# edouardlp/Mask-RCNN-CoreML

Hardware: AMD Instinct MI355X
Metric: images/sec (1024x1024, COCO-80) (higher is better)
Workload: dtype f32x3

## Files before the change

### mask-rcnn-coreml_amd/csrc/kernels_conv_halo.hip

```cpp
#include "conv_device.h"

#include <stdlib.h>
#include <map>
#include <mutex>
#include <string>
#include <utility>

namespace mrcnn {

ConvScratch* conv_current_scratch();

static int env_int_halo(const char* name, int dflt) { const char* e = knob_env(name); return e ? atoi(e) : dflt; }

static constexpr int HALO_MAX_SLOT = 640;
static constexpr unsigned HALO_OOB = 0xC0000000u;
enum { HALO_GEO_LINEAR = 0,
       HALO_GEO_ROW = 1,
       HALO_GEO_2ROWS = 2,
       HALO_GEO_4ROWS = 3 };

typedef unsigned u32x4 __attribute__((ext_vector_type(4)));
typedef unsigned u32x2 __attribute__((ext_vector_type(2)));

struct HaloArgs {
    ConvArgs a;
    const void* wgt_halo;
    int NH;
    int geo;
    int ecols;
    int pitch;
    int img_skew;
    int tiles_row, tiles_img;
    int n_tiles;
    const void* head_w;
    const float* head_bias;
    float* head_out; float* head_out2;
    long head_out_sB, head_out_sP, head_out2_sB, head_out2_sP;
    int head_split, head_cols;
    float head_mul;
    ConvArgs t;
    const void* t_w;
    void* t_park;
};

template <int PARTS>
__device__ __forceinline__ void split4(const u32x4 v, u32x2 (&out)[PARTS])
{
    const float a[4] = {__uint_as_float(v[0]), __uint_as_float(v[1]), __uint_as_float(v[2]), __uint_as_float(v[3])};
#pragma unroll
    for (int p = 0; p < 2; ++p) {
        const uint32_t h2 = cvt_pk_rne(a[2 * p], a[2 * p + 1]);
        float r0, r1;
        asm("v_fma_mix_f32 %0, %1, -1.0, %2 op_sel:[0,0,0] op_sel_hi:[1,0,0]" : "=v"(r0) : "v"(h2), "v"(a[2 * p]));
        asm("v_fma_mix_f32 %0, %1, -1.0, %2 op_sel:[1,0,0] op_sel_hi:[1,0,0]" : "=v"(r1) : "v"(h2), "v"(a[2 * p + 1]));
        const uint32_t m2 = cvt_pk_rne(r0, r1);
        out[0][p] = h2;
        out[1][p] = m2;
        if constexpr (PARTS == 3) {
            float q0, q1;
            asm("v_fma_mix_f32 %0, %1, -1.0, %2 op_sel:[0,0,0] op_sel_hi:[1,0,0]" : "=v"(q0) : "v"(m2), "v"(r0));
            asm("v_fma_mix_f32 %0, %1, -1.0, %2 op_sel:[1,0,0] op_sel_hi:[1,0,0]" : "=v"(q1) : "v"(m2), "v"(r1));
            out[2][p] = cvt_pk_rne(q0, q1);
        }
    }
}

template <int PARTS, int TN, bool HEAD = false, bool DBG = false, int TM = 2, int MAXPC = 5, bool TAIL = false, int WN = 4>
__global__ __launch_bounds__(512, 2) void k_conv_halo(const HaloArgs ha)
{
    const ConvArgs& a = ha.a;
    static_assert(WN == 4 || (WN == 2 && TM == 1 && TN == 1 && !HEAD && !TAIL) || (WN == 1 && TM == 1 && TN == 2 && !HEAD && !TAIL),
                  "wave arrangement 2 x 4; 4 x 2 with one accumulator per wave; 8 x 1 with two (256 x 64 tiles)");
    static_assert(!HEAD || TN == 2, "the fused head walks the K groups of 256-column tiles");
    static_assert(!TAIL || (TM == 2 && TN == 2 && !HEAD), "the fused tail needs the whole 128 x 256 tile in one block");
    static_assert(MAXPC >= 2 && MAXPC <= 5, "staging pieces per thread");
    constexpr int WMR = 8 / WN;
    constexpr int BM = WMR * TM * 32, BN = WN * TN * 32;
    constexpr int PLANE = (HALO_MAX_SLOT + 1) * 32;
    constexpr int PBUF = PARTS * PLANE;
    constexpr int STAGE = 8 * 32 * 36 * 4;
    constexpr int HPART = 4 * BM * 32 * 4;
    constexpr int HRUN = HEAD ? BM * 32 * 4 : 0;
    constexpr int PLANES_ = 2 * PBUF > PBUF + STAGE ? 2 * PBUF : PBUF + STAGE;
    constexpr int TAILPL = 16 * 64 * 32;
    constexpr int TAILN = 1024;
    constexpr int TPLANES = TAIL ? PARTS * TAILPL + STAGE : 0;
    constexpr int PLANES__ = HEAD && HPART > PLANES_ ? HPART : PLANES_;
    constexpr int PLANES = TPLANES > PLANES__ ? TPLANES : PLANES__;
    constexpr int TAB1 = TAIL ? 2 * TAILN * 4 : 0;
    __shared__ __attribute__((aligned(16))) unsigned char smem[PLANES + 2 * 2 * BN * 4 + HRUN + TAB1];
    unsigned char* const planes = smem;
    float* const s_tab0 = reinterpret_cast<float*>(smem + PLANES);
    float* const h_run = reinterpret_cast<float*>(smem + PLANES + 2 * 2 * BN * 4);
    float* const tab1 = reinterpret_cast<float*>(smem + PLANES + 2 * 2 * BN * 4 + HRUN);

    const int t = threadIdx.x;
    const int lane = t & 63;
    const int wave = __builtin_amdgcn_readfirstlane(t >> 6);
    const int wm = WN == 4 ? wave >> 2 : (WN == 2 ? wave >> 1 : wave), wn = WN == 4 ? wave & 3 : (WN == 2 ? wave & 1 : 0);
    const int l31 = lane & 31, kk = lane >> 5;
    const int ohw = a.OH * a.OW;
    const int NH = ha.NH, NS = NH * 9;

    const int T = HEAD ? a.tiles_m : ha.n_tiles;
    const int n_inner = HEAD ? a.tiles_n : 1;
    const int nb = gridDim.x;
    const int bid = blockIdx.x;
    int t_first, t_end, t_step;
    {
        const int q = T >> 3, r8 = T & 7;
        const int xcd = bid & 7, j = bid >> 3;
        const int lo = xcd < r8 ? xcd * (q + 1) : r8 * (q + 1) + (xcd - r8) * q;
        const int cnt = q + (xcd < r8 ? 1 : 0);
        const int per = nb >> 3;
        t_first = lo + j; t_end = lo + cnt; t_step = per;
        if (nb < 8) { t_first = bid; t_end = T; t_step = nb; }
    }

    typedef unsigned srd_t __attribute__((ext_vector_type(4)));
    srd_t srdB;
    {
        const unsigned long long wa = (unsigned long long)(uintptr_t)ha.wgt_halo;
        srdB[0] = __builtin_amdgcn_readfirstlane((unsigned)wa);
        srdB[1] = __builtin_amdgcn_readfirstlane((unsigned)(wa >> 32) & 0xffffu);
        srdB[2] = 0xffffffffu;
        srdB[3] = 0x00020000u;
    }
    const unsigned vlane16 = (unsigned)lane * 16u;
    srd_t srdT;
    {
        const unsigned long long ta_ = (unsigned long long)(uintptr_t)(TAIL ? ha.t_w : ha.wgt_halo);
        srdT[0] = __builtin_amdgcn_readfirstlane((unsigned)ta_);
        srdT[1] = __builtin_amdgcn_readfirstlane((unsigned)(ta_ >> 32) & 0xffffu);
        srdT[2] = 0xffffffffu;
        srdT[3] = 0x00020000u;
    }
    if constexpr (TAIL) {
        const float4 one = make_float4(1.f, 1.f, 1.f, 1.f), zero = make_float4(0.f, 0.f, 0.f, 0.f);
        if (t < TAILN / 4) {
            *reinterpret_cast<float4*>(&tab1[4 * t]) = ha.t.scale ? *reinterpret_cast<const float4*>(ha.t.scale + 4 * t) : one;
            *reinterpret_cast<float4*>(&tab1[TAILN + 4 * t]) = ha.t.shift ? *reinterpret_cast<const float4*>(ha.t.shift + 4 * t) : zero;
        }
    }
    const int dbg = DBG ? a.dbg : 0;
    const bool dbg_nodma = dbg & 1, dbg_nobar = dbg & 2, dbg_nords = dbg & 4, dbg_nomma = dbg & 8, dbg_nostage = dbg & 16;
    const bool dbg_noloads = dbg & 64, dbg_nosplit = dbg & 128, dbg_nowrite = dbg & 256;

    int tile_par = 0;
    for (int unit = t_first; unit < t_end; unit += t_step)
    for (int inner = 0; inner < n_inner; ++inner, tile_par ^= 1) {
        const int mt = HEAD ? unit : unit / a.tiles_n, nt = HEAD ? inner : unit - mt * a.tiles_n;
        const int n0 = nt * BN;
        float* const s_tab = s_tab0 + tile_par * 2 * BN;
        const int Hp = a.H + 2;
        const int pitch = ha.pitch, ecols = ha.ecols;
        int m0, b0, gy_first, col0, rows;
        if (ha.geo == HALO_GEO_2ROWS || ha.geo == HALO_GEO_4ROWS) {
            const int trows = ha.geo == HALO_GEO_2ROWS ? 2 : 4;
            b0 = mt / ha.tiles_img;
            const int r = mt - b0 * ha.tiles_img, rp = r / ha.tiles_row, cb = r - rp * ha.tiles_row;
            m0 = b0 * ohw + trows * rp * a.OW + 64 * cb;
            gy_first = b0 * Hp + trows * rp + 1;
            col0 = 64 * cb - 1;
            rows = trows + 2;
        } else {
            m0 = mt * BM;
            const int m_last = (m0 + BM - 1 < a.M ? m0 + BM - 1 : a.M - 1);
            b0 = m0 / ohw;
            const int rem0 = m0 - b0 * ohw, oh0 = rem0 / a.OW, ow0 = rem0 - oh0 * a.OW;
            const int b1 = m_last / ohw, rem1 = m_last - b1 * ohw, oh1 = rem1 / a.OW;
            gy_first = b0 * Hp + oh0 + 1;
            const int gy_last = b1 * Hp + oh1 + 1;
            col0 = ha.geo == HALO_GEO_ROW ? ow0 - 1 : -1;
            rows = gy_last - gy_first + 3;
        }
        const int npx = rows * ecols;
        srd_t srdA;
        {
            const unsigned long long ia = (unsigned long long)(uintptr_t)(static_cast<const float*>(a.in) + (long)b0 * a.in_sB);
            const unsigned long long rest = (unsigned long long)(a.B - b0) * (unsigned long long)a.in_sB * 4ull;
            srdA[0] = __builtin_amdgcn_readfirstlane((unsigned)ia);
            srdA[1] = __builtin_amdgcn_readfirstlane((unsigned)(ia >> 32) & 0xffffu);
            srdA[2] = __builtin_amdgcn_readfirstlane((unsigned)(rest < 0x80000000ull ? rest : 0x80000000ull));
            srdA[3] = 0x00020000u;
        }
        unsigned p_off[MAXPC], p_lds[MAXPC];
#pragma unroll
        for (int i = 0; i < MAXPC; ++i) {
            const int j = t + 512 * i;
            const int px = j >> 2, qt = j & 3;
            const int r = px / ecols, c = px - r * ecols;
            const int gy = gy_first - 1 + r;
            const int b = gy / Hp, y = gy - b * Hp - 1;
            const int x = col0 + c;
            const bool ok = px < npx && (unsigned)y < (unsigned)a.H && (unsigned)x < (unsigned)a.W && b < a.B;
            p_off[i] = ok ? (unsigned)(((long)(b - b0) * a.in_sB + (long)y * a.in_sH + (long)x * a.in_sW + qt * 4) * 4) : HALO_OOB;
            if (DBG && (a.dbg & 32)) p_off[i] = (unsigned)((px & 63) * 1024 + qt * 16);
            const int slot = r * pitch + c + (b - b0) * ha.img_skew;
            p_lds[i] = px < npx ? (unsigned)(slot * 32 + (((qt >> 1) ^ ((slot >> 3) & 1)) << 4) + (qt & 1) * 8) : (unsigned)(HALO_MAX_SLOT * 32 + qt * 8);
        }
        int base_idx[TM];
        int wave_row0;
        if (ha.geo == HALO_GEO_2ROWS || ha.geo == HALO_GEO_4ROWS) {
            if constexpr (WN == 4) {
                wave_row0 = m0 + wm * a.OW;
#pragma unroll
                for (int i = 0; i < TM; ++i) base_idx[i] = wm * pitch + i * 32 + l31;
            } else {
                wave_row0 = m0 + (wm >> 1) * a.OW + (wm & 1) * 32;
                base_idx[0] = (wm >> 1) * pitch + (wm & 1) * 32 + l31;
            }
        } else {
            wave_row0 = m0 + wm * (TM * 32);
            const int ow0 = col0 + 1;
#pragma unroll
            for (int i = 0; i < TM; ++i) {
                const int m = wave_row0 + i * 32 + l31;
                const int mm = m < a.M ? m : a.M - 1;
                const int b = mm / ohw, rem = mm - b * ohw, oh = rem / a.OW, ow = rem - oh * a.OW;
                base_idx[i] = ha.geo == HALO_GEO_ROW ? (ow - ow0) : (b * Hp + oh + 1 - gy_first) * pitch + ow + (b - b0) * ha.img_skew;
            }
        }
        unsigned sob[TN];
#pragma unroll
        for (int j = 0; j < TN; ++j) sob[j] = (unsigned)(((size_t)(n0 / 32 + wn * TN + j) * NS) * 1024u);

        if (t < BN / 2) {
            const int c = (t < BN / 4 ? t : t - BN / 4) * 4;
            const float* src = t < BN / 4 ? a.scale : a.shift;
            const float fill = t < BN / 4 ? 1.0f : 0.0f;
            *reinterpret_cast<float4*>(&s_tab[(t < BN / 4 ? 0 : BN) + c]) =
                src ? *reinterpret_cast<const float4*>(src + n0 + c) : make_float4(fill, fill, fill, fill);
        }

#define HALO_LOAD(I) if constexpr ((I) < MAXPC) asm volatile("buffer_load_dwordx4 %0, %1, %2, 0 offen" : "=v"(st[(I) < MAXPC ? (I) : 0]) : "v"(p_off[(I) < MAXPC ? (I) : 0]), "s"(srdA) : "memory");
#define HALO_LOADS()  { HALO_LOAD(0) HALO_LOAD(1) HALO_LOAD(2) HALO_LOAD(3) HALO_LOAD(4) }
#define HALO_ADVANCE() { _Pragma("unroll") for (int i = 0; i < MAXPC; ++i) p_off[i] += (p_off[i] < HALO_OOB ? 64u : 0u); }
#define HALO_PIN1(I)  if constexpr ((I) < MAXPC) asm volatile("" : "+v"(st[(I) < MAXPC ? (I) : 0]));
#define HALO_PIN()    { HALO_PIN1(0) HALO_PIN1(1) HALO_PIN1(2) HALO_PIN1(3) HALO_PIN1(4) }
#define HALO_WRITE1(BUF, I_)                                                                                     \
    if constexpr ((I_) < MAXPC) {                                                                                \
        constexpr int I = (I_) < MAXPC ? (I_) : 0;                                                               \
        u32x2 parts[PARTS];                                                                                      \
        if (DBG && dbg_nosplit) { _Pragma("unroll") for (int p = 0; p < PARTS; ++p) { parts[p][0] = st[I][0]; parts[p][1] = st[I][p]; } } \
        else split4<PARTS>(st[I], parts);                                                                        \
        if (DBG && dbg_nowrite) { _Pragma("unroll") for (int p = 0; p < PARTS; ++p) asm volatile("" ::"v"(parts[p])); } \
        else {                                                                                                   \
            _Pragma("unroll") for (int p = 0; p < PARTS; ++p)                                                    \
                *reinterpret_cast<u32x2*>(planes + (BUF) * PBUF + p * PLANE + p_lds[I]) = parts[p];              \
        }                                                                                                        \
    }
#define HALO_WRITE(BUF) { HALO_WRITE1(BUF, 0) HALO_WRITE1(BUF, 1) HALO_WRITE1(BUF, 2) HALO_WRITE1(BUF, 3) HALO_WRITE1(BUF, 4) }
#define HALO_BLOAD(BV, STEP_)                                                                                    \
    {                                                                                                            \
        _Pragma("unroll") for (int j = 0; j < TN; ++j) {                                                         \
            const unsigned so_ = sob[j] + (unsigned)(STEP_) * 1024u;                                             \
            asm volatile("buffer_load_dwordx4 %0, %1, %2, %3 offen" : "=v"(BV[j]) : "v"(vlane16), "s"(srdB), "s"(so_) : "memory"); \
        }                                                                                                        \
    }
#define HALO_BPIN(BV) { _Pragma("unroll") for (int j = 0; j < TN; ++j) asm volatile("" : "+v"(BV[j])); }
        u32x4 st[MAXPC];
        u32x4 bv0[TN], bv1[TN], bv2[TN], bv3[TN];

        HALO_LOADS()
        HALO_ADVANCE()
        HALO_BLOAD(bv0, 0)
        HALO_BLOAD(bv1, 1)
        HALO_BLOAD(bv2, 2)
        asm volatile("s_waitcnt vmcnt(0)" ::: "memory");
        HALO_PIN()
        HALO_BPIN(bv0)
        HALO_BPIN(bv1)
        HALO_BPIN(bv2)
        HALO_WRITE(0)
        __syncthreads();

        f32x16 acc[TM][TN];
#pragma unroll
        for (int i = 0; i < TM; ++i)
#pragma unroll
            for (int j = 0; j < TN; ++j)
#pragma unroll
                for (int e = 0; e < 16; ++e) acc[i][j][e] = 0.0f;

#define HALO_AFRAGS(AV, PB_, TAP_)                                                                               \
    {                                                                                                            \
        _Pragma("unroll") for (int i = 0; i < TM; ++i) {                                                         \
            const int idx_ = base_idx[i] + ((TAP_) / 3) * pitch + ((TAP_) % 3);                                  \
            const unsigned a_addr_ = (unsigned)(idx_ << 5) + (unsigned)(((kk << 4) ^ ((idx_ << 1) & 16)));       \
            _Pragma("unroll") for (int p = 0; p < PARTS; ++p) AV[i][p] = *reinterpret_cast<const uint4*>(planes + (PB_) * PBUF + p * PLANE + a_addr_); \
        }                                                                                                        \
    }
#define HALO_STEP(BVC, BVN3, TAP, PB)                                                                            \
    {                                                                                                            \
          \
        if (!(DBG && dbg_nodma)) HALO_BLOAD(BVN3, step + 3 < NS ? step + 3 : NS - 1)                             \
        if ((TAP) == 0 && next_slab && !(DBG && dbg_noloads)) { HALO_LOADS() HALO_ADVANCE() }                    \
        if (!(DBG && dbg_nomma)) {                                                                               \
        _Pragma("unroll") for (int p = 0; p < PARTS; ++p)                                                        \
            _Pragma("unroll") for (int i = 0; i < TM; ++i)                                                       \
                _Pragma("unroll") for (int j = 0; j < TN; ++j)                                                   \
                    acc[i][j] = __builtin_amdgcn_mfma_f32_32x32x16_f16(__builtin_bit_cast(f16x8, BVC[j]), __builtin_bit_cast(f16x8, av[i][p]), acc[i][j], 0, 0, 0); \
        }                                                                                                        \
                                 \
        if (!(DBG && dbg_nords)) {                                                                               \
            if ((TAP) == 8) HALO_AFRAGS(av, (PB) ^ 1, 0)                                                         \
            else HALO_AFRAGS(av, PB, ((TAP) + 1) % 9)                                                            \
        }                                                                                                        \
            \
        if ((TAP) == 4 && next_slab) { HALO_PIN() HALO_WRITE1((PB) ^ 1, 0) HALO_WRITE1((PB) ^ 1, 4) }            \
        if ((TAP) == 5 && next_slab) HALO_WRITE1((PB) ^ 1, 1)                                                    \
        if ((TAP) == 6 && next_slab) HALO_WRITE1((PB) ^ 1, 2)                                                    \
        if ((TAP) == 7 && next_slab) HALO_WRITE1((PB) ^ 1, 3)                                                    \
        if (DBG && (dbg_nodma || dbg_noloads)) asm volatile("s_waitcnt vmcnt(0)" ::: "memory");                  \
        else if ((TAP) <= 2 && next_slab) asm volatile("s_waitcnt vmcnt(%0)" ::"n"(2 * TN + MAXPC) : "memory");  \
        else asm volatile("s_waitcnt vmcnt(%0)" ::"n"(2 * TN) : "memory");                                       \
        HALO_BPIN(bv0) HALO_BPIN(bv1) HALO_BPIN(bv2) HALO_BPIN(bv3)                                              \
        if ((TAP) == 7 && !(DBG && dbg_nobar)) __syncthreads();                                                  \
        ++step;                                                                                                  \
    }
#define HALO_SLAB(B0, B1, B2, B3, PB)                                                                            \
    HALO_STEP(B0, B3, 0, PB) HALO_STEP(B1, B0, 1, PB) HALO_STEP(B2, B1, 2, PB) HALO_STEP(B3, B2, 3, PB) HALO_STEP(B0, B3, 4, PB) \
    HALO_STEP(B1, B0, 5, PB) HALO_STEP(B2, B1, 6, PB) HALO_STEP(B3, B2, 7, PB) HALO_STEP(B0, B3, 8, PB)
        uint4 av[TM][PARTS];
        HALO_AFRAGS(av, 0, 0)
        int step = 0;
        for (int h = 0; h < NH; h += 4) {
            { const bool next_slab = !dbg_nostage;                 HALO_SLAB(bv0, bv1, bv2, bv3, 0) }
            { const bool next_slab = !dbg_nostage;                 HALO_SLAB(bv1, bv2, bv3, bv0, 1) }
            { const bool next_slab = !dbg_nostage;                 HALO_SLAB(bv2, bv3, bv0, bv1, 0) }
            { const bool next_slab = h + 4 < NH && !dbg_nostage;   HALO_SLAB(bv3, bv0, bv1, bv2, 1) }
        }
        asm volatile("s_waitcnt vmcnt(0)" ::: "memory");
        HALO_BPIN(bv0) HALO_BPIN(bv1) HALO_BPIN(bv2) HALO_BPIN(bv3)
#undef HALO_SLAB
#undef HALO_STEP
#undef HALO_AFRAGS
#undef HALO_BPIN
#undef HALO_BLOAD
#undef HALO_WRITE
#undef HALO_WRITE1
#undef HALO_PIN
#undef HALO_PIN1
#undef HALO_ADVANCE
#undef HALO_LOADS
#undef HALO_LOAD
        if constexpr (TAIL) {
            const ConvArgs& t1 = ha.t;
            unsigned char* const tpl = smem;
            float* const tstage = reinterpret_cast<float*>(smem + PARTS * TAILPL) + wave * (32 * 36);
            const bool relu3 = a.act == ACT_RELU;
            bool oor = false;
            if (t1.dbg & 4) { if (acc[0][0][0] == 123.456f) tab1[1] = acc[1][1][3]; continue; }
            float4* const park = static_cast<float4*>(ha.t_park) + ((size_t)blockIdx.x * 4 + wn) * 16 * 64 + lane;
            auto stage_piece = [&](const float (&x)[4], int i, int j, int q) {
                u32x4 v = {__float_as_uint(x[0]), __float_as_uint(x[1]), __float_as_uint(x[2]), __float_as_uint(x[3])};
                u32x2 parts[PARTS];
                split4<PARTS>(v, parts);
                const int row = i * 32 + l31, g = wn * 4 + j * 2 + (q >> 1);
                const unsigned addr = (unsigned)((g * 64 + row) * 32 + ((((q & 1) ^ (row >> 3)) & 1) << 4) + 8 * kk);
#pragma unroll
                for (int p = 0; p < PARTS; ++p) *reinterpret_cast<u32x2*>(tpl + p * TAILPL + addr) = parts[p];
            };
            __syncthreads();
            if (!(t1.dbg & 8))
#pragma unroll
            for (int i = 0; i < TM; ++i)
#pragma unroll
                for (int j = 0; j < TN; ++j)
#pragma unroll
                    for (int q = 0; q < 4; ++q) {
                        const int cl = wn * 64 + j * 32 + 8 * q + 4 * kk;
                        const float4 sc = *reinterpret_cast<const float4*>(s_tab + cl), sh = *reinterpret_cast<const float4*>(s_tab + BN + cl);
                        float x[4] = {acc[i][j][4 * q + 0] * sc.x + sh.x, acc[i][j][4 * q + 1] * sc.y + sh.y,
                                      acc[i][j][4 * q + 2] * sc.z + sh.z, acc[i][j][4 * q + 3] * sc.w + sh.w};
#pragma unroll
                        for (int r = 0; r < 4; ++r) {
                            if (relu3) x[r] = fmaxf(x[r], 0.f);
                            oor = oor || !(fabsf(x[r]) < 65504.0f);
                        }
                        if (wm == 0) stage_piece(x, i, j, q);
                        else park[((i * 2 + j) * 4 + q) * 64] = make_float4(x[0], x[1], x[2], x[3]);
                    }
            if (a.range_flag && oor) atomicOr(a.range_flag, 1);
#pragma unroll 1
            for (int h = 0; h < 2; ++h) {
                if (h == 1 && wm == 1 && !(t1.dbg & 8)) {
#pragma unroll
                    for (int i = 0; i < TM; ++i)
#pragma unroll
                        for (int j = 0; j < TN; ++j)
#pragma unroll
                            for (int q = 0; q < 4; ++q) {
                                const float4 y = park[((i * 2 + j) * 4 + q) * 64];
                                const float x[4] = {y.x, y.y, y.z, y.w};
                                stage_piece(x, i, j, q);
                            }
                }
                __syncthreads();
                const int half_row0 = ha.geo == HALO_GEO_2ROWS ? m0 + h * a.OW : m0 + h * 64;
#pragma unroll 1
                for (int it = 0; it < 2; ++it) {
                    const int n1 = it * 512 + wave * 64;
                    f32x16 acc1[2][2];
#pragma unroll
                    for (int i = 0; i < 2; ++i)
#pragma unroll
                        for (int j = 0; j < 2; ++j)
#pragma unroll
                            for (int e = 0; e < 16; ++e) acc1[i][j][e] = 0.0f;
                    const unsigned wofs = (unsigned)((n1 / 32) * 16 * 1024);
                    u32x4 bw[3][2];
#define TAIL_BLOAD(SET, S_)                                                                                      \
    {                                                                                                            \
// ... 8 lines not shown
                    const unsigned a_off = (unsigned)(l31 * 32 + ((kk ^ ((l31 >> 3) & 1)) << 4));
                    uint4 fa[2][PARTS];
#pragma unroll
                    for (int i = 0; i < 2; ++i)
#pragma unroll
                        for (int p = 0; p < PARTS; ++p) fa[i][p] = *reinterpret_cast<const uint4*>(tpl + p * TAILPL + (i * 32) * 32 + a_off);
                    asm volatile("s_waitcnt vmcnt(2)" ::: "memory");
                    TAIL_BPIN()
#pragma unroll
                    for (int s = 0; s < 16; ++s) {
                        if (t1.dbg & 2) { asm volatile("s_waitcnt vmcnt(0)" ::: "memory"); break; }
                        if (s + 2 < 16) TAIL_BLOAD((s + 2) % 3, s + 2)
#pragma unroll
                        for (int i = 0; i < 2; ++i)
#pragma unroll
                            for (int p = 0; p < PARTS; ++p)
#pragma unroll
                                for (int j = 0; j < 2; ++j)
                                    acc1[i][j] = __builtin_amdgcn_mfma_f32_32x32x16_f16(__builtin_bit_cast(f16x8, bw[s % 3][j]), __builtin_bit_cast(f16x8, fa[i][p]),
                                                                                        acc1[i][j], 0, 0, 0);
                        if (s + 1 < 16) {
#pragma unroll
                            for (int i = 0; i < 2; ++i)
#pragma unroll
                                for (int p = 0; p < PARTS; ++p)
                                    fa[i][p] = *reinterpret_cast<const uint4*>(tpl + p * TAILPL + ((s + 1) * 64 + i * 32) * 32 + a_off);
                        }
                        if (s + 2 < 16) asm volatile("s_waitcnt vmcnt(2)" ::: "memory");
                        else asm volatile("s_waitcnt vmcnt(0)" ::: "memory");
                        TAIL_BPIN()
                    }
#undef TAIL_BPIN
#undef TAIL_BLOAD
                    if (!(t1.dbg & 1))
                        conv_epilogue_wave<TAILN, 2, 2, true>(t1, acc1, tstage, tab1, half_row0, 0, n1, lane);
                    else if (acc1[0][0][0] == 123.456f) tab1[0] = acc1[1][1][3];
                }
                __syncthreads();
            }
        } else if constexpr (!HEAD) {
            conv_epilogue_wave<BN, TM, TN>(a, acc, reinterpret_cast<float*>(planes + PBUF) + wave * (32 * 36), s_tab, wave_row0, n0,
                                           wn * TN * 32, lane);
        } else {
            const bool relu = a.act == ACT_RELU;
            bool out_of_range = false;
            f32x16 hp[TM];
#pragma unroll
            for (int i = 0; i < TM; ++i)
#pragma unroll
                for (int e = 0; e < 16; ++e) hp[i][e] = 0.0f;
            const unsigned hw_off = (unsigned)(((n0 + wn * TN * 32) / 16) * 1024);
#pragma unroll
            for (int j = 0; j < TN; ++j)
#pragma unroll
                for (int g = 0; g < 2; ++g) {
                    const uint4 wf = *reinterpret_cast<const uint4*>(static_cast<const char*>(ha.head_w) + hw_off + (j * 2 + g) * 1024 + lane * 16);
#pragma unroll
                    for (int i = 0; i < TM; ++i) {
                        u32x4 v0, v1;
#pragma unroll
                        for (int q2 = 0; q2 < 2; ++q2) {
                            const int cl = wn * TN * 32 + j * 32 + 8 * (2 * g + q2) + 4 * kk;
                            const float4 sc = *reinterpret_cast<const float4*>(s_tab + cl), sh = *reinterpret_cast<const float4*>(s_tab + BN + cl);
                            float x[4] = {acc[i][j][8 * g + 4 * q2 + 0] * sc.x + sh.x, acc[i][j][8 * g + 4 * q2 + 1] * sc.y + sh.y,
                                          acc[i][j][8 * g + 4 * q2 + 2] * sc.z + sh.z, acc[i][j][8 * g + 4 * q2 + 3] * sc.w + sh.w};
#pragma unroll
                            for (int r = 0; r < 4; ++r) {
                                if (relu) x[r] = fmaxf(x[r], 0.f);
                                out_of_range = out_of_range || !(fabsf(x[r]) < 65504.0f);
                                if (q2 == 0) v0[r] = __float_as_uint(x[r]); else v1[r] = __float_as_uint(x[r]);
                            }
                        }
                        u32x2 p0[PARTS], p1[PARTS];
                        split4<PARTS>(v0, p0);
                        split4<PARTS>(v1, p1);
#pragma unroll
                        for (int p = 0; p < PARTS; ++p) {
                            const u32x4 af = {p0[p][0], p0[p][1], p1[p][0], p1[p][1]};
                            hp[i] = __builtin_amdgcn_mfma_f32_32x32x16_f16(__builtin_bit_cast(f16x8, wf), __builtin_bit_cast(f16x8, af), hp[i], 0, 0, 0);
                        }
                    }
                }
            if (a.range_flag && out_of_range) atomicOr(a.range_flag, 1);
            float* const part = reinterpret_cast<float*>(planes);
#pragma unroll
            for (int i = 0; i < TM; ++i)
#pragma unroll
                for (int q = 0; q < 4; ++q)
                    *reinterpret_cast<float4*>(&part[((wn * BM) + wm * (TM * 32) + i * 32 + l31) * 32 + (((2 * q + kk) ^ (l31 & 7)) << 2)]) =
                        make_float4(hp[i][4 * q], hp[i][4 * q + 1], hp[i][4 * q + 2], hp[i][4 * q + 3]);
            __syncthreads();
            const bool last = inner == n_inner - 1;
#pragma unroll
            for (int k = 0; k < BM / 16; ++k) {
                const int o = t + 512 * k, row = o >> 5, col = o & 31;
                float sum = inner == 0 ? 0.0f : h_run[o];
                const int pc = ((((col >> 2) ^ (row & 7)) << 2) | (col & 3));
                sum += part[(0 * BM + row) * 32 + pc];
                sum += part[(1 * BM + row) * 32 + pc];
                sum += part[(2 * BM + row) * 32 + pc];
                sum += part[(3 * BM + row) * 32 + pc];
                if (!last) h_run[o] = sum;
                else {
                    const int m = ha.geo == HALO_GEO_2ROWS ? m0 + (row >> 6) * a.OW + (row & 63) : m0 + row;
                    if (m < a.M && col < ha.head_cols) {
                        const float y = sum * ha.head_mul + ha.head_bias[col];
                        const int b = m / ohw, pix = m - b * ohw;
                        if (col < ha.head_split) ha.head_out[(long)b * ha.head_out_sB + (long)pix * ha.head_out_sP + col] = y;
                        else ha.head_out2[(long)b * ha.head_out2_sB + (long)pix * ha.head_out2_sP + (col - ha.head_split)] = y;
                    }
                }
            }
            __syncthreads();
        }
    }
}

static constexpr int HALO_LAT_MAX_SLOT = 320;
template <int PARTS, int MAXPC>
__global__ __launch_bounds__(256, 2) void k_conv_halo_lat(const HaloArgs ha)
{
    const ConvArgs& a = ha.a;
    static_assert(MAXPC >= 3 && MAXPC <= 5, "staging pieces per thread");
    constexpr int BM = 64, BN = 64, NT = 256, D = 11, NSET = 12;
    constexpr int PLANE = (HALO_LAT_MAX_SLOT + 1) * 32;
    constexpr int PBUF = PARTS * PLANE;
    static_assert(PBUF >= 4 * 32 * 32 * 4, "the four wave-private epilogue tiles live in plane buffer 1");
    __shared__ __attribute__((aligned(16))) unsigned char smem[2 * PBUF + 2 * 2 * BN * 4];
    unsigned char* const planes = smem;
    float* const s_tab0 = reinterpret_cast<float*>(smem + 2 * PBUF);

    const int t = threadIdx.x;
    const int lane = t & 63;
    const int wave = __builtin_amdgcn_readfirstlane(t >> 6);
    const int wm = wave >> 1, wn = wave & 1;
    const int l31 = lane & 31, kk = lane >> 5;
    const int ohw = a.OH * a.OW;
    const int NH = ha.NH, NS = NH * 9;

    const int T = ha.n_tiles;
    const int nb = gridDim.x;
    const int bid = blockIdx.x;
    int t_first, t_end, t_step;
    {
        const int q = T >> 3, r8 = T & 7;
        const int xcd = bid & 7, j = bid >> 3;
        const int lo = xcd < r8 ? xcd * (q + 1) : r8 * (q + 1) + (xcd - r8) * q;
        const int cnt = q + (xcd < r8 ? 1 : 0);
        const int per = nb >> 3;
        t_first = lo + j; t_end = lo + cnt; t_step = per;
        if (nb < 8) { t_first = bid; t_end = T; t_step = nb; }
    }
    typedef unsigned srd_t __attribute__((ext_vector_type(4)));
    srd_t srdB;
    {
        const unsigned long long wa = (unsigned long long)(uintptr_t)ha.wgt_halo;
        srdB[0] = __builtin_amdgcn_readfirstlane((unsigned)wa);
        srdB[1] = __builtin_amdgcn_readfirstlane((unsigned)(wa >> 32) & 0xffffu);
        srdB[2] = 0xffffffffu;
        srdB[3] = 0x00020000u;
    }
    const unsigned vlane16 = (unsigned)lane * 16u;

    int tile_par = 0;
    for (int unit = t_first; unit < t_end; unit += t_step, tile_par ^= 1) {
        const int mt = unit / a.tiles_n, nt = unit - mt * a.tiles_n;
        const int n0 = nt * BN;
        float* const s_tab = s_tab0 + tile_par * 2 * BN;
        const int Hp = a.H + 2;
        const int pitch = ha.pitch, ecols = ha.ecols;
        const int m0 = mt * BM;
        const int m_last = (m0 + BM - 1 < a.M ? m0 + BM - 1 : a.M - 1);
        const int b0 = m0 / ohw;
        const int rem0 = m0 - b0 * ohw, oh0 = rem0 / a.OW, ow0 = rem0 - oh0 * a.OW;
        const int b1 = m_last / ohw, rem1 = m_last - b1 * ohw, oh1 = rem1 / a.OW;
        const int gy_first = b0 * Hp + oh0 + 1;
        const int gy_last = b1 * Hp + oh1 + 1;
        const int col0 = ha.geo == HALO_GEO_ROW ? ow0 - 1 : -1;
        const int rows = gy_last - gy_first + 3;
        const int npx = rows * ecols;
        srd_t srdA;
        {
            const unsigned long long ia = (unsigned long long)(uintptr_t)(static_cast<const float*>(a.in) + (long)b0 * a.in_sB);
            const unsigned long long rest = (unsigned long long)(a.B - b0) * (unsigned long long)a.in_sB * 4ull;
            srdA[0] = __builtin_amdgcn_readfirstlane((unsigned)ia);
            srdA[1] = __builtin_amdgcn_readfirstlane((unsigned)(ia >> 32) & 0xffffu);
            srdA[2] = __builtin_amdgcn_readfirstlane((unsigned)(rest < 0x80000000ull ? rest : 0x80000000ull));
            srdA[3] = 0x00020000u;
        }
        unsigned p_off[MAXPC], p_lds[MAXPC];
#pragma unroll
        for (int i = 0; i < MAXPC; ++i) {
            const int j = t + NT * i;
            const int px = j >> 2, qt = j & 3;
            const int r = px / ecols, c = px - r * ecols;
            const int gy = gy_first - 1 + r;
            const int b = gy / Hp, y = gy - b * Hp - 1;
// ... 108 lines not shown
            { const bool stage_now = h + 5 < NH && LAT_ABL(8), write_next = h + 4 < NH && LAT_ABL(8), stage_prev = h + 4 < NH && LAT_ABL(8);           LAT_SLAB(27, 1, 1) }
        }
        asm volatile("s_waitcnt vmcnt(0)" ::: "memory");
        LAT_BPIN()
#undef LAT_SLAB
#undef LAT_STEP
#undef LAT_MFMA
#undef LAT_PIECE
#undef LAT_AFRAGS
#undef LAT_BARRIER
#undef LAT_BPIN
#undef LAT_BLOAD
#undef LAT_WRITE1
#undef LAT_PIN
#undef LAT_PIN1
#undef LAT_ADVANCE
#undef LAT_LOADS
#undef LAT_LOAD
        f32x16 accs[1][1];
        accs[0][0] = acc;
        if (!LAT_ABL(16)) { if (acc[0] == 123.456f) s_tab[0] = acc[3]; continue; }
        conv_epilogue_wave<BN, 1, 1>(a, accs, reinterpret_cast<float*>(planes + PBUF) + wave * (32 * 32), s_tab, wave_row0, n0, wn * 32, lane);
#undef LAT_ABL
    }
}

__global__ __launch_bounds__(256) void k_halo_pack(const uint4* __restrict__ src, int Npad, int Cin, int taps, uint4* __restrict__ dst)
{
    const int NH = Cin / 16;
    const long total = (long)(Npad / 32) * NH * taps * 64;
    for (long e = (long)blockIdx.x * 256 + threadIdx.x; e < total; e += (long)gridDim.x * 256) {
        const int piece = (int)(e & 63);
        const long gs = e >> 6;
        const int step = (int)(gs % (NH * taps));
        const int g = (int)(gs / (NH * taps));
        const int h = step / taps, tap = step - h * taps;
        const int r = piece & 31, half = piece >> 5;
        const int n = g * 32 + r;
        dst[e] = src[(((long)n * taps + tap) * Cin + 16 * h + 8 * half) / 8];
    }
}

__global__ __launch_bounds__(256) void k_halo_pack_head(const uint16_t* __restrict__ src, int Cin, uint16_t* __restrict__ dst)
{
    const long total = (long)(Cin / 16) * 64 * 8;
    for (long e = (long)blockIdx.x * 256 + threadIdx.x; e < total; e += (long)gridDim.x * 256) {
        const int sl = (int)(e & 7), lane = (int)((e >> 3) & 63);
        const int G = (int)(e >> 9);
        const int n = lane & 31, kk = lane >> 5;
        dst[e] = src[(long)n * Cin + 16 * G + 4 * kk + (sl & 3) + 8 * (sl >> 2)];
    }
}

void conv_halo_pack_head(hipStream_t s, const void* wgt_std, int Npad, int Cin, DevBuf& out)
{
    MRCNN_REQUIRE(Npad == 32 && Cin % 16 == 0, MRCNN_ERR_SHAPE, "halo head packing: Npad %d (must be 32) / Cin %d", Npad, Cin);
    out.alloc((size_t)32 * Cin * 2);
    hipLaunchKernelGGL(k_halo_pack_head, dim3(64), dim3(256), 0, s, static_cast<const uint16_t*>(wgt_std), Cin, static_cast<uint16_t*>(out.p));
    HIP_CHECK(hipGetLastError());
}

void conv_halo_pack(hipStream_t s, const void* wgt_std, int Npad, int Cin, DevBuf& out, int taps)
{
    MRCNN_REQUIRE(Npad % 32 == 0 && Cin % 16 == 0 && (taps == 9 || taps == 1), MRCNN_ERR_SHAPE, "halo packing: Npad %d / Cin %d / taps %d", Npad, Cin, taps);
    const size_t bytes = (size_t)Npad * taps * Cin * 2;
    out.alloc(bytes);
    const long total = (long)bytes / 16;
    const int grid = (int)((total + 255) / 256 < 4096 ? (total + 255) / 256 : 4096);
    hipLaunchKernelGGL(k_halo_pack, dim3(grid), dim3(256), 0, s, static_cast<const uint4*>(wgt_std), Npad, Cin, taps, static_cast<uint4*>(out.p));
    HIP_CHECK(hipGetLastError());
}

static int halo_linear_rows(int H, int W, int bm)
{
    const int rows_touched = (bm - 1 + W - 1) / W + 1;
    const long ohw = (long)H * W;
    const int boundaries = ohw % bm == 0 ? 0 : (int)((bm - 1 + ohw - 1) / ohw);
    return rows_touched + 2 * boundaries + 2;
}

static int g_halo_lat = env_int_halo("MRCNN_HALO_LAT", 1);
static int g_halo_rounds = env_int_halo("MRCNN_HALO_ROUNDS", 1);
static int g_halo_n64 = env_int_halo("MRCNN_HALO_N64", 2);
static int g_halo_geo = env_int_halo("MRCNN_HALO_GEO", 1);

struct HaloGeo { int geo, ecols, pitch, img_skew, tiles_row, tiles_img, rows, maxpc, slots; bool ok; };

static HaloGeo halo_geometry(int H, int W, int bm)
{
    HaloGeo g{};
    int slots_extra = 0;
    if (g_halo_geo == 0) {
        const bool row = W % 128 == 0;
        g.geo = row ? HALO_GEO_ROW : HALO_GEO_LINEAR;
        g.ecols = g.pitch = row ? 130 : W + 2;
        g.rows = row ? 3 : halo_linear_rows(H, W, bm);
        g.maxpc = 5;
        g.ok = g.rows * g.ecols <= 528;
        return g;
    }
    if (bm == 256) {
        if (W % 64 != 0 || H % 4 != 0) return g;
        g.geo = HALO_GEO_4ROWS; g.ecols = g.pitch = 66; g.rows = 6;
        g.tiles_row = W / 64; g.tiles_img = (H / 4) * g.tiles_row;
    } else if (bm == 128 && W % 64 == 0 && W >= 128 && H % 2 == 0) {
        g.geo = HALO_GEO_2ROWS; g.ecols = g.pitch = 66; g.rows = 4;
        g.tiles_row = W / 64; g.tiles_img = (H / 2) * g.tiles_row;
    } else if (W % bm == 0) {
        g.geo = HALO_GEO_ROW; g.ecols = g.pitch = bm + 2; g.rows = 3;
    } else {
        g.geo = HALO_GEO_LINEAR; g.ecols = W + 2; g.rows = halo_linear_rows(H, W, bm);
        g.pitch = W % 32 == 0 ? W + 2 : W + 16;
        const long ohw = (long)H * W;
        const int boundaries = ohw % bm == 0 ? 0 : (int)((bm - 1 + ohw - 1) / ohw);
        g.img_skew = g.pitch == W + 16 ? (16 - (2 * W) % 16) % 16 : 0;
        if (g.rows * g.pitch + boundaries * g.img_skew > HALO_MAX_SLOT) { g.pitch = W + 2; g.img_skew = 0; }
        slots_extra = boundaries * g.img_skew;
    }
    const int px = g.rows * g.ecols;
    g.maxpc = px <= 256 ? 2 : px <= 384 ? 3 : 5;
    g.slots = g.rows * g.pitch + slots_extra;
    g.ok = px <= 640 && g.slots <= HALO_MAX_SLOT;
    return g;
}

bool conv_halo_eligible(const ConvDesc& d)
{
    const int wdtype = d.wdtype < 0 ? d.dtype : d.wdtype;
    const bool split = d.dtype == MRCNN_F32 && (wdtype == MRCNN_F16 || wdtype == MRCNN_F32X3);
    if (!split || d.KH != 3 || d.KW != 3 || d.stride != 1 || d.padH != 1 || d.padW != 1) return false;
    if (d.OH != d.H || d.OW != d.W || d.Cin % 64 != 0 || (d.Npad % 128 != 0 && !(d.Npad == 64 && g_halo_n64)) || d.Cout % 4 != 0) return false;
    if (d.deconv2 || d.out2 || d.sel_partial || d.act == ACT_SIGMOID || d.res) return false;
    if (d.H >= 32760 || d.W >= 32760 || (double)d.in_sB * 8.0 >= 2.0e9) return false;
    const bool legacy_ok = (d.W % 128 == 0 ? 3 * 130 : halo_linear_rows(d.H, d.W, 128) * (d.W + 2)) <= 528;
    if (g_halo_geo == 0) return legacy_ok;
    const bool rows2_ok = d.W % 64 == 0 && d.H % 2 == 0;
    return (legacy_ok || rows2_ok) && halo_geometry(d.H, d.W, 128).ok && halo_geometry(d.H, d.W, 64).ok;
}

template <int PARTS, int TN, bool HEAD, int TM>
static void halo_launch_pc(hipStream_t s, const HaloArgs& ha, int maxpc, int grid)
{
    if (maxpc == 2) {
        if constexpr (!HEAD) hipLaunchKernelGGL((k_conv_halo<PARTS, TN, HEAD, false, TM, 2>), dim3(grid), dim3(512), 0, s, ha);
        else hipLaunchKernelGGL((k_conv_halo<PARTS, TN, HEAD, false, TM, 3>), dim3(grid), dim3(512), 0, s, ha);
    } else if (maxpc == 3) hipLaunchKernelGGL((k_conv_halo<PARTS, TN, HEAD, false, TM, 3>), dim3(grid), dim3(512), 0, s, ha);
    else hipLaunchKernelGGL((k_conv_halo<PARTS, TN, HEAD, false, TM, 5>), dim3(grid), dim3(512), 0, s, ha);
}

template <int PARTS>
static void halo_launch(hipStream_t s, const HaloArgs& ha, int bm, int bn, int maxpc, int grid)
{
    if (ha.a.dbg && !ha.head_w && bn == 256 && PARTS == 3) {
        if (maxpc <= 3) hipLaunchKernelGGL((k_conv_halo<3, 2, false, true, 2, 3>), dim3(grid), dim3(512), 0, s, ha);
        else hipLaunchKernelGGL((k_conv_halo<3, 2, false, true, 2, 5>), dim3(grid), dim3(512), 0, s, ha);
        return;
    }
    if (bn == 64 && bm == 256) {
        hipLaunchKernelGGL((k_conv_halo<PARTS, 2, false, false, 1, 5, false, 1>), dim3(grid), dim3(512), 0, s, ha);
        return;
    }
    if (bn == 64) {
        if (maxpc == 2) hipLaunchKernelGGL((k_conv_halo<PARTS, 1, false, false, 1, 2, false, 2>), dim3(grid), dim3(512), 0, s, ha);
        else if (maxpc == 3) hipLaunchKernelGGL((k_conv_halo<PARTS, 1, false, false, 1, 3, false, 2>), dim3(grid), dim3(512), 0, s, ha);
        else hipLaunchKernelGGL((k_conv_halo<PARTS, 1, false, false, 1, 5, false, 2>), dim3(grid), dim3(512), 0, s, ha);
        return;
    }
    if (ha.head_w && bm == 64) hipLaunchKernelGGL((k_conv_halo<PARTS, 2, true, false, 1, 3>), dim3(grid), dim3(512), 0, s, ha);
    else if (ha.head_w) halo_launch_pc<PARTS, 2, true, 2>(s, ha, maxpc, grid);
    else if (bn == 256) halo_launch_pc<PARTS, 2, false, 2>(s, ha, maxpc, grid);
    else if (bm == 128) halo_launch_pc<PARTS, 1, false, 2>(s, ha, maxpc, grid);
    else halo_launch_pc<PARTS, 1, false, 1>(s, ha, maxpc, grid);
}

bool conv_halo_packable(int KH, int KW, int Cin, int Npad) { return KH == 3 && KW == 3 && Cin % 64 == 0 && (Npad % 128 == 0 || Npad == 64); }

bool conv_halo_debug_set(const char* key, int value)
{
    if (std::string(key) == "halo_geo") { g_halo_geo = value; return true; }
    if (std::string(key) == "halo_lat") { g_halo_lat = value; return true; }
    if (std::string(key) == "halo_n64") { g_halo_n64 = value; return true; }
    if (std::string(key) == "halo_rounds") { g_halo_rounds = value; return true; }
    return false;
}

bool conv_halo_head_eligible(const ConvDesc& d)
{
    return conv_halo_eligible(d) && d.Npad % 256 == 0 && d.Npad == d.Cout && ((long)d.OH * d.OW) % 128 == 0 && (long)d.OH * d.OW >= 4096 &&
           d.head_cols >= 1 && d.head_cols <= 32 && d.head_split >= 0 && d.head_split <= d.head_cols;
}

bool conv_halo_tail_packable(int KH, int KW, int Cin, int Npad) { return KH == 1 && KW == 1 && Cin == 256 && Npad == 1024; }
bool conv_halo_tail_geometry_ok(int H, int W) { const HaloGeo g = halo_geometry(H, W, 128); return g.ok && g.maxpc <= 3; }

int conv_halo_forward(hipStream_t s, ConvArgs a, const ConvDesc& d, int parts, int n_cus, const ConvArgs* t1, const void* t_w)
{
    HaloArgs ha;
    ha.t_w = t_w;
    ha.t_park = nullptr;
    if (t1) ha.t = *t1;
    int bm = 128, bn = d.Npad % 256 == 0 ? 256 : (d.Npad % 128 == 0 ? 128 : 64);
    if (bn == 64 && g_halo_n64 >= 2 && g_halo_geo && halo_geometry(d.H, d.W, 256).ok && (long)(a.M / 256) >= (long)n_cus * 2) bm = 256;
    if (!d.head_w && !t1 && bn != 64) {
        if (bn > 128 && (long)((a.M + 127) / 128) * (d.Npad / bn) < n_cus) bn = 128;
        if (bn == 128 && (long)((a.M + 127) / 128) * (d.Npad / bn) * 4 < (long)n_cus * 3) bm = 64;
        if (bn == 128 && bm == 128 && g_halo_rounds) {
            const long t128 = (long)((a.M + 127) / 128) * (d.Npad / bn), t64 = (long)((a.M + 63) / 64) * (d.Npad / bn);
            const long r128 = (t128 + n_cus - 1) / n_cus, r64 = (t64 + n_cus - 1) / n_cus;
            if (r64 * 575 < r128 * 1000 && halo_geometry(d.H, d.W, 64).ok) bm = 64;
        }
    }
    if (d.head_w && (long)((a.M + 127) / 128) * 4 < (long)n_cus * 3 && d.W % 64 == 0) bm = 64;
    MRCNN_REQUIRE(!t1 || (bn == 256 && d.Npad == 256), MRCNN_ERR_INVALID, "fused tail: the 3x3 layer must have exactly 256 output columns");
    int lat_pc = 0;
    if (!d.head_w && !t1 && g_halo_lat && g_halo_geo && bm == 64 && bn == 128 && (long)((a.M + 63) / 64) * (d.Npad / 128) * 8 < (long)n_cus * 3 * g_halo_lat) {
        const HaloGeo g64 = halo_geometry(d.H, d.W, 64);
        const int px = g64.rows * g64.ecols;
        if (g64.ok && g64.geo != HALO_GEO_2ROWS && px <= 320 && g64.slots <= HALO_LAT_MAX_SLOT) { lat_pc = px <= 192 ? 3 : px <= 256 ? 4 : 5; bn = 64; }
    }
    const int tiles_m = (a.M + bm - 1) / bm;
    a.tiles_m = tiles_m;
    a.tiles_n = d.Npad / bn;
    a.direct = 1;
    ha.a = a;
    ha.wgt_halo = d.wgt_halo;
    ha.NH = d.Cin / 16;
    const HaloGeo g = halo_geometry(d.H, d.W, bm);
    MRCNN_REQUIRE(g.ok, MRCNN_ERR_SHAPE, "halo kernel: no tile geometry for %dx%d (conv_halo_eligible should have said so)", d.H, d.W);
    ha.geo = g.geo; ha.ecols = g.ecols; ha.pitch = g.pitch; ha.img_skew = g.img_skew; ha.tiles_row = g.tiles_row; ha.tiles_img = g.tiles_img;
    ha.n_tiles = a.tiles_m * a.tiles_n;
    ha.head_w = d.head_w; ha.head_bias = d.head_bias; ha.head_out = d.head_out; ha.head_out2 = d.head_out2;
    ha.head_out_sB = d.head_out_sB; ha.head_out_sP = d.head_out_sP; ha.head_out2_sB = d.head_out2_sB; ha.head_out2_sP = d.head_out2_sP;
    ha.head_split = d.head_split; ha.head_cols = d.head_cols; ha.head_mul = d.head_mul;
    const int units = d.head_w ? a.tiles_m : ha.n_tiles;
    int grid = units < n_cus ? units : n_cus;
    if (grid >= 8) grid &= ~7;
    if (t1) {
        ha.t.direct = 1;
        {
            ConvScratch* const sc = conv_current_scratch();
            MRCNN_REQUIRE(sc, MRCNN_ERR_INVALID, "fused tail without a ConvScratch (conv_forward_tail checks)");
            if (sc->park.bytes < (size_t)grid * 65536) {
                hipStreamCaptureStatus cap = hipStreamCaptureStatusNone;
                HIP_CHECK(hipStreamIsCapturing(s, &cap));
                MRCNN_REQUIRE(cap == hipStreamCaptureStatusNone, MRCNN_ERR_INVALID, "fused tail: the parking buffer must exist before a stream capture (run the predict once eagerly)");
                HIP_CHECK(hipStreamSynchronize(s));
                sc->park.alloc((size_t)grid * 65536);
            }
            ha.t_park = sc->park.p;
        }
        MRCNN_REQUIRE(g.maxpc <= 3, MRCNN_ERR_INVALID, "fused tail: the tile's input region needs more than three staging pieces (conv_halo_tail_geometry_ok)");
        if (parts == 3) hipLaunchKernelGGL((k_conv_halo<3, 2, false, false, 2, 3, true>), dim3(grid), dim3(512), 0, s, ha);
        else hipLaunchKernelGGL((k_conv_halo<2, 2, false, false, 2, 3, true>), dim3(grid), dim3(512), 0, s, ha);
        return bn;
    }
    if (lat_pc) {
        grid = units < 2 * n_cus ? units : 2 * n_cus;
        if (grid >= 8) grid &= ~7;
#define MRCNN_LAT(P, PC) hipLaunchKernelGGL((k_conv_halo_lat<P, PC>), dim3(grid), dim3(256), 0, s, ha)
        if (parts == 3) { if (lat_pc == 3) MRCNN_LAT(3, 3); else if (lat_pc == 4) MRCNN_LAT(3, 4); else MRCNN_LAT(3, 5); }
        else { if (lat_pc == 3) MRCNN_LAT(2, 3); else if (lat_pc == 4) MRCNN_LAT(2, 4); else MRCNN_LAT(2, 5); }
#undef MRCNN_LAT
        return bn;
    }
    if (parts == 3) halo_launch<3>(s, ha, bm, bn, g.maxpc, grid);
    else halo_launch<2>(s, ha, bm, bn, g.maxpc, grid);
    return bn;
}

}
```

Baseline: 444.7.

## Carry the next tile's input staging and weight prefetch across persistent-kernel tile boundaries

In the persistent halo conv kernel, the last K group of each tile now prefetches the next tile's weights and stages its first input slab, so the next tile skips its cold prologue (loads, waitcnt, LDS write). Each tile's staging geometry is computed through a helper, and the fused-head partial buffer moves past the carried plane to avoid clobbering it. This removes per-tile pipeline drain and refill at the cost of more LDS in the head variant, extra register pressure from weight registers kept live across tiles, and more complex control flow. A grid-cap knob is also added but is off by default.

Result: no change. 443.7 (-0.2%).

```diff
diff --git a/mask-rcnn-coreml_amd/csrc/kernels_conv_halo.hip b/mask-rcnn-coreml_amd/csrc/kernels_conv_halo.hip
--- a/mask-rcnn-coreml_amd/csrc/kernels_conv_halo.hip
+++ b/mask-rcnn-coreml_amd/csrc/kernels_conv_halo.hip
@@ -32,6 +32,7 @@
     int img_skew;
     int tiles_row, tiles_img;
     int n_tiles;
+    int carry;
     const void* head_w;
     const float* head_bias;
     float* head_out; float* head_out2;
@@ -74,6 +75,7 @@
     static_assert(!HEAD || TN == 2, "the fused head walks the K groups of 256-column tiles");
     static_assert(!TAIL || (TM == 2 && TN == 2 && !HEAD), "the fused tail needs the whole 128 x 256 tile in one block");
     static_assert(MAXPC >= 2 && MAXPC <= 5, "staging pieces per thread");
+    constexpr bool CARRY = !TAIL && !DBG && !(HEAD && MAXPC == 5);
     constexpr int WMR = 8 / WN;
     constexpr int BM = WMR * TM * 32, BN = WN * TN * 32;
     constexpr int PLANE = (HALO_MAX_SLOT + 1) * 32;
@@ -85,7 +87,8 @@
     constexpr int TAILPL = 16 * 64 * 32;
     constexpr int TAILN = 1024;
     constexpr int TPLANES = TAIL ? PARTS * TAILPL + STAGE : 0;
-    constexpr int PLANES__ = HEAD && HPART > PLANES_ ? HPART : PLANES_;
+    constexpr int HPOFF = CARRY ? PBUF : 0;
+    constexpr int PLANES__ = HEAD && HPOFF + HPART > PLANES_ ? HPOFF + HPART : PLANES_;
     constexpr int PLANES = TPLANES > PLANES__ ? TPLANES : PLANES__;
     constexpr int TAB1 = TAIL ? 2 * TAILN * 4 : 0;
     __shared__ __attribute__((aligned(16))) unsigned char smem[PLANES + 2 * 2 * BN * 4 + HRUN + TAB1];
@@ -146,36 +149,37 @@
     const bool dbg_nodma = dbg & 1, dbg_nobar = dbg & 2, dbg_nords = dbg & 4, dbg_nomma = dbg & 8, dbg_nostage = dbg & 16;
     const bool dbg_noloads = dbg & 64, dbg_nosplit = dbg & 128, dbg_nowrite = dbg & 256;
 
-    int tile_par = 0;
-    for (int unit = t_first; unit < t_end; unit += t_step)
-    for (int inner = 0; inner < n_inner; ++inner, tile_par ^= 1) {
-        const int mt = HEAD ? unit : unit / a.tiles_n, nt = HEAD ? inner : unit - mt * a.tiles_n;
-        const int n0 = nt * BN;
-        float* const s_tab = s_tab0 + tile_par * 2 * BN;
-        const int Hp = a.H + 2;
-        const int pitch = ha.pitch, ecols = ha.ecols;
-        int m0, b0, gy_first, col0, rows;
+    const int Hp = a.H + 2;
+    const int pitch = ha.pitch, ecols = ha.ecols;
+    struct Region { int m0, b0, gy_first, col0, rows; };
+    auto region_of = [&](const int mt) -> Region {
+        Region g;
         if (ha.geo == HALO_GEO_2ROWS || ha.geo == HALO_GEO_4ROWS) {
             const int trows = ha.geo == HALO_GEO_2ROWS ? 2 : 4;
-            b0 = mt / ha.tiles_img;
-            const int r = mt - b0 * ha.tiles_img, rp = r / ha.tiles_row, cb = r - rp * ha.tiles_row;
-            m0 = b0 * ohw + trows * rp * a.OW + 64 * cb;
-            gy_first = b0 * Hp + trows * rp + 1;
-            col0 = 64 * cb - 1;
-            rows = trows + 2;
+            g.b0 = mt / ha.tiles_img;
+            const int r = mt - g.b0 * ha.tiles_img, rp = r / ha.tiles_row, cb = r - rp * ha.tiles_row;
+            g.m0 = g.b0 * ohw + trows * rp * a.OW + 64 * cb;
+            g.gy_first = g.b0 * Hp + trows * rp + 1;
+            g.col0 = 64 * cb - 1;
+            g.rows = trows + 2;
         } else {
-            m0 = mt * BM;
-            const int m_last = (m0 + BM - 1 < a.M ? m0 + BM - 1 : a.M - 1);
-            b0 = m0 / ohw;
-            const int rem0 = m0 - b0 * ohw, oh0 = rem0 / a.OW, ow0 = rem0 - oh0 * a.OW;
+            g.m0 = mt * BM;
+            const int m_last = (g.m0 + BM - 1 < a.M ? g.m0 + BM - 1 : a.M - 1);
+            g.b0 = g.m0 / ohw;
+            const int rem0 = g.m0 - g.b0 * ohw, oh0 = rem0 / a.OW, ow0 = rem0 - oh0 * a.OW;
             const int b1 = m_last / ohw, rem1 = m_last - b1 * ohw, oh1 = rem1 / a.OW;
-            gy_first = b0 * Hp + oh0 + 1;
+            g.gy_first = g.b0 * Hp + oh0 + 1;
             const int gy_last = b1 * Hp + oh1 + 1;
-            col0 = ha.geo == HALO_GEO_ROW ? ow0 - 1 : -1;
-            rows = gy_last - gy_first + 3;
-        }
-        const int npx = rows * ecols;
-        srd_t srdA;
+            g.col0 = ha.geo == HALO_GEO_ROW ? ow0 - 1 : -1;
+            g.rows = gy_last - g.gy_first + 3;
+        }
+        return g;
+    };
+    srd_t srdA;
+    unsigned p_off[MAXPC], p_lds[MAXPC];
+    auto stage_geometry = [&](const Region& g) {
+        const int npx = g.rows * ecols;
+        const int b0 = g.b0;
         {
             const unsigned long long ia = (unsigned long long)(uintptr_t)(static_cast<const float*>(a.in) + (long)b0 * a.in_sB);
             const unsigned long long rest = (unsigned long long)(a.B - b0) * (unsigned long long)a.in_sB * 4ull;
@@ -184,21 +188,39 @@
             srdA[2] = __builtin_amdgcn_readfirstlane((unsigned)(rest < 0x80000000ull ? rest : 0x80000000ull));
             srdA[3] = 0x00020000u;
         }
-        unsigned p_off[MAXPC], p_lds[MAXPC];
 #pragma unroll
         for (int i = 0; i < MAXPC; ++i) {
             const int j = t + 512 * i;
             const int px = j >> 2, qt = j & 3;
             const int r = px / ecols, c = px - r * ecols;
-            const int gy = gy_first - 1 + r;
+            const int gy = g.gy_first - 1 + r;
             const int b = gy / Hp, y = gy - b * Hp - 1;
-            const int x = col0 + c;
+            const int x = g.col0 + c;
             const bool ok = px < npx && (unsigned)y < (unsigned)a.H && (unsigned)x < (unsigned)a.W && b < a.B;
             p_off[i] = ok ? (unsigned)(((long)(b - b0) * a.in_sB + (long)y * a.in_sH + (long)x * a.in_sW + qt * 4) * 4) : HALO_OOB;
             if (DBG && (a.dbg & 32)) p_off[i] = (unsigned)((px & 63) * 1024 + qt * 16);
             const int slot = r * pitch + c + (b - b0) * ha.img_skew;
             p_lds[i] = px < npx ? (unsigned)(slot * 32 + (((qt >> 1) ^ ((slot >> 3) & 1)) << 4) + (qt & 1) * 8) : (unsigned)(HALO_MAX_SLOT * 32 + qt * 8);
         }
+    };
+    const bool carry_on = CARRY && ha.carry != 0;
+    bool carried = false;
+    u32x4 bv0[TN], bv1[TN], bv2[TN], bv3[TN];
+
+    int tile_par = 0;
+    for (int unit = t_first; unit < t_end; unit += t_step)
+    for (int inner = 0; inner < n_inner; ++inner, tile_par ^= 1) {
+        const int mt = HEAD ? unit : unit / a.tiles_n, nt = HEAD ? inner : unit - mt * a.tiles_n;
+        const int n0 = nt * BN;
+        float* const s_tab = s_tab0 + tile_par * 2 * BN;
+        const bool same_m = HEAD && inner + 1 < n_inner;
+        const int unit_n = same_m ? unit : unit + t_step;
+        const int mt_n = HEAD ? unit_n : unit_n / a.tiles_n;
+        const int n0_n = (HEAD ? (same_m ? inner + 1 : 0) : unit_n - mt_n * a.tiles_n) * BN;
+        const bool carry_next = carry_on && unit_n < t_end;
+        const Region rg = region_of(mt);
+        const int m0 = rg.m0, b0 = rg.b0, gy_first = rg.gy_first, col0 = rg.col0;
+        if (!carried) stage_geometry(rg);
         int base_idx[TM];
         int wave_row0;
         if (ha.geo == HALO_GEO_2ROWS || ha.geo == HALO_GEO_4ROWS) {
@@ -224,6 +246,11 @@
         unsigned sob[TN];
 #pragma unroll
         for (int j = 0; j < TN; ++j) sob[j] = (unsigned)(((size_t)(n0 / 32 + wn * TN + j) * NS) * 1024u);
+        unsigned sob_past[TN];
+        const unsigned past_mul = carry_next ? 1024u : 0u;
+#pragma unroll
+        for (int j = 0; j < TN; ++j)
+            sob_past[j] = carry_next ? (unsigned)(((size_t)(n0_n / 32 + wn * TN + j) * NS) * 1024u) : sob[j] + (unsigned)(NS - 1) * 1024u;
 
         if (t < BN / 2) {
             const int c = (t < BN / 4 ? t : t - BN / 4) * 4;
@@ -254,25 +281,26 @@
 #define HALO_BLOAD(BV, STEP_)                                                                                    \
     {                                                                                                            \
         _Pragma("unroll") for (int j = 0; j < TN; ++j) {                                                         \
-            const unsigned so_ = sob[j] + (unsigned)(STEP_) * 1024u;                                             \
+            const unsigned so_ = (STEP_) < NS ? sob[j] + (unsigned)(STEP_) * 1024u : sob_past[j] + (unsigned)((STEP_) - NS) * past_mul; \
             asm volatile("buffer_load_dwordx4 %0, %1, %2, %3 offen" : "=v"(BV[j]) : "v"(vlane16), "s"(srdB), "s"(so_) : "memory"); \
         }                                                                                                        \
     }
 #define HALO_BPIN(BV) { _Pragma("unroll") for (int j = 0; j < TN; ++j) asm volatile("" : "+v"(BV[j])); }
         u32x4 st[MAXPC];
-        u32x4 bv0[TN], bv1[TN], bv2[TN], bv3[TN];
-
-        HALO_LOADS()
-        HALO_ADVANCE()
-        HALO_BLOAD(bv0, 0)
-        HALO_BLOAD(bv1, 1)
-        HALO_BLOAD(bv2, 2)
-        asm volatile("s_waitcnt vmcnt(0)" ::: "memory");
-        HALO_PIN()
-        HALO_BPIN(bv0)
-        HALO_BPIN(bv1)
-        HALO_BPIN(bv2)
-        HALO_WRITE(0)
+
+        if (!carried) {
+            HALO_LOADS()
+            HALO_ADVANCE()
+            HALO_BLOAD(bv0, 0)
+            HALO_BLOAD(bv1, 1)
+            HALO_BLOAD(bv2, 2)
+            asm volatile("s_waitcnt vmcnt(0)" ::: "memory");
+            HALO_PIN()
+            HALO_BPIN(bv0)
+            HALO_BPIN(bv1)
+            HALO_BPIN(bv2)
+            HALO_WRITE(0)
+        }
         __syncthreads();
 
         f32x16 acc[TM][TN];
@@ -293,8 +321,8 @@
     }
 #define HALO_STEP(BVC, BVN3, TAP, PB)                                                                            \
     {                                                                                                            \
-          \
-        if (!(DBG && dbg_nodma)) HALO_BLOAD(BVN3, step + 3 < NS ? step + 3 : NS - 1)                             \
+                                                                             \
+        if (!(DBG && dbg_nodma)) HALO_BLOAD(BVN3, step + 3)                                                      \
         if ((TAP) == 0 && next_slab && !(DBG && dbg_noloads)) { HALO_LOADS() HALO_ADVANCE() }                    \
         if (!(DBG && dbg_nomma)) {                                                                               \
         _Pragma("unroll") for (int p = 0; p < PARTS; ++p)                                                        \
@@ -329,7 +357,14 @@
             { const bool next_slab = !dbg_nostage;                 HALO_SLAB(bv0, bv1, bv2, bv3, 0) }
             { const bool next_slab = !dbg_nostage;                 HALO_SLAB(bv1, bv2, bv3, bv0, 1) }
             { const bool next_slab = !dbg_nostage;                 HALO_SLAB(bv2, bv3, bv0, bv1, 0) }
-            { const bool next_slab = h + 4 < NH && !dbg_nostage;   HALO_SLAB(bv3, bv0, bv1, bv2, 1) }
+            const bool last_group = h + 4 >= NH;
+            if (CARRY && last_group && carry_next) {
+                if (same_m) {
+#pragma unroll
+                    for (int i = 0; i < MAXPC; ++i) p_off[i] -= (p_off[i] < HALO_OOB ? 64u * (unsigned)NH : 0u);
+                } else stage_geometry(region_of(mt_n));
+            }
+            { const bool next_slab = (!last_group || carry_next) && !dbg_nostage;   HALO_SLAB(bv3, bv0, bv1, bv2, 1) }
         }
         asm volatile("s_waitcnt vmcnt(0)" ::: "memory");
         HALO_BPIN(bv0) HALO_BPIN(bv1) HALO_BPIN(bv2) HALO_BPIN(bv3)
@@ -504,7 +539,7 @@
                     }
                 }
             if (a.range_flag && out_of_range) atomicOr(a.range_flag, 1);
-            float* const part = reinterpret_cast<float*>(planes);
+            float* const part = reinterpret_cast<float*>(planes + HPOFF);
 #pragma unroll
             for (int i = 0; i < TM; ++i)
 #pragma unroll
@@ -535,6 +570,7 @@
             }
             __syncthreads();
         }
+        carried = carry_next;
     }
 }
 
@@ -809,6 +845,8 @@
 static int g_halo_lat = env_int_halo("MRCNN_HALO_LAT", 1);
 static int g_halo_rounds = env_int_halo("MRCNN_HALO_ROUNDS", 1);
 static int g_halo_n64 = env_int_halo("MRCNN_HALO_N64", 2);
+static int g_halo_carry = env_int_halo("MRCNN_HALO_CARRY", 1);
+static int g_halo_grid_cap = env_int_halo("MRCNN_HALO_GRID_CAP", 0);
 static int g_halo_geo = env_int_halo("MRCNN_HALO_GEO", 1);
 
 struct HaloGeo { int geo, ecols, pitch, img_skew, tiles_row, tiles_img, rows, maxpc, slots; bool ok; };
@@ -905,6 +943,8 @@
 bool conv_halo_debug_set(const char* key, int value)
 {
     if (std::string(key) == "halo_geo") { g_halo_geo = value; return true; }
+    if (std::string(key) == "halo_carry") { g_halo_carry = value; return true; }
+    if (std::string(key) == "halo_grid_cap") { g_halo_grid_cap = value; return true; }
     if (std::string(key) == "halo_lat") { g_halo_lat = value; return true; }
     if (std::string(key) == "halo_n64") { g_halo_n64 = value; return true; }
     if (std::string(key) == "halo_rounds") { g_halo_rounds = value; return true; }
@@ -961,7 +1001,9 @@
     ha.head_split = d.head_split; ha.head_cols = d.head_cols; ha.head_mul = d.head_mul;
     const int units = d.head_w ? a.tiles_m : ha.n_tiles;
     int grid = units < n_cus ? units : n_cus;
+    if (g_halo_grid_cap > 0 && grid > g_halo_grid_cap) grid = g_halo_grid_cap;
     if (grid >= 8) grid &= ~7;
+    ha.carry = g_halo_carry;
     if (t1) {
         ha.t.direct = 1;
         {
```
